# commaai/rednose

Measured on NVIDIA H100. Metric: fused EKF predict+update steps/s (batched, float64), higher is better.
Workload: dtype f64

## Files before the change

### rednose_b200/build.py

```python
import os
import shutil
import subprocess

PKG_DIR = os.path.dirname(os.path.abspath(__file__))
CSRC_DIR = os.path.join(PKG_DIR, "csrc")
INCLUDE_DIR = os.path.abspath(os.path.join(PKG_DIR, "..", "include"))
GENERATED_DIR = os.environ.get("REDNOSE_B200_GENERATED_DIR") or os.path.join(PKG_DIR, "generated")

NVCC_FLAGS = [
  "-gencode", "arch=compute_90a,code=sm_90a",
  "-O3", "-lineinfo", "-std=c++17", "--expt-relaxed-constexpr",
  "-Xcompiler", "-fPIC", "-shared",
]


def nvcc_path():
  p = shutil.which("nvcc") or "/usr/local/cuda/bin/nvcc"
  if not os.path.exists(p):
    raise RuntimeError("nvcc not found: rednose_b200 needs the CUDA toolkit to build filter libraries")
  return p


TUNE_ENV = ("REDNOSE_B200_GROUP", "REDNOSE_B200_WARPS", "REDNOSE_B200_TMA", "REDNOSE_B200_STAGES", "REDNOSE_B200_TMA_STORE", "REDNOSE_B200_SMALLSYM",
            "REDNOSE_B200_RTS_MMA", "REDNOSE_B200_MIN_WARPS", "REDNOSE_B200_PAIR", "REDNOSE_B200_PAIR_GROUP", "REDNOSE_B200_PAIR_MIN_WARPS",
            "REDNOSE_B200_RTS_MIN_CTAS", "REDNOSE_B200_CTA_MIN_BLOCKS", "REDNOSE_B200_PAIR_WAR_FIX", "REDNOSE_B200_PAIR_LATE_REFILL", "REDNOSE_B200_MAXRREG")


def _flags_match(folder, name):
  want = " ".join(f"{e}={os.environ[e]}" for e in TUNE_ENV if os.environ.get(e))
  try:
    with open(os.path.join(folder, f".{name}.env"), encoding="utf-8") as f:
      return f.read() == want
  except OSError:
    return want == ""


def _newer(target, sources):
  if not os.path.exists(target):
    return False
  t = os.path.getmtime(target)
  return all(os.path.getmtime(s) <= t for s in sources if os.path.exists(s))


def csrc_sources():
  return [os.path.join(CSRC_DIR, f) for f in sorted(os.listdir(CSRC_DIR)) if f != "runtime.cc"] + [os.path.join(INCLUDE_DIR, "rednose_b200.h")]


def compile_filter(folder, name, force=False, verbose=False):
  src = os.path.join(folder, f"{name}.cu")
  lib = os.path.join(folder, f"lib{name}.so")
  if not force and _newer(lib, [src] + csrc_sources()) and _flags_match(folder, name):
    return lib
  import fcntl
  with open(os.path.join(folder, f".{name}.lock"), "w") as lock:
    fcntl.flock(lock, fcntl.LOCK_EX)
    if not force and _newer(lib, [src] + csrc_sources()) and _flags_match(folder, name):
      return lib
    out = _compile_filter_locked(folder, name, src, lib, verbose)
    with open(os.path.join(folder, f".{name}.env"), "w", encoding="utf-8") as f:
      f.write(" ".join(f"{e}={os.environ[e]}" for e in TUNE_ENV if os.environ.get(e)))
    return out


def _compile_filter_locked(folder, name, src, lib, verbose):
  tune = [f"-D{k}={os.environ[e]}" for k, e in (("RNB_GROUP", "REDNOSE_B200_GROUP"), ("RNB_WARPS", "REDNOSE_B200_WARPS"), ("RNB_TMA", "REDNOSE_B200_TMA"), ("RNB_STAGES", "REDNOSE_B200_STAGES"), ("RNB_TMA_STORE", "REDNOSE_B200_TMA_STORE"), ("RNB_SMALLSYM", "REDNOSE_B200_SMALLSYM"), ("RNB_RTS_MMA", "REDNOSE_B200_RTS_MMA"), ("RNB_MIN_WARPS", "REDNOSE_B200_MIN_WARPS"), ("RNB_PAIR", "REDNOSE_B200_PAIR"), ("RNB_PAIR_GROUP", "REDNOSE_B200_PAIR_GROUP"), ("RNB_PAIR_MIN_WARPS", "REDNOSE_B200_PAIR_MIN_WARPS"), ("RNB_RTS_MIN_CTAS", "REDNOSE_B200_RTS_MIN_CTAS"), ("RNB_CTA_MIN_BLOCKS", "REDNOSE_B200_CTA_MIN_BLOCKS"), ("RNB_PAIR_WAR_FIX", "REDNOSE_B200_PAIR_WAR_FIX"), ("RNB_PAIR_LATE_REFILL", "REDNOSE_B200_PAIR_LATE_REFILL")) if os.environ.get(e)]
  if os.environ.get("REDNOSE_B200_MAXRREG"):
    tune += ["-maxrregcount", os.environ["REDNOSE_B200_MAXRREG"]]
  tmp = lib + f".tmp{os.getpid()}"
  cmd = [nvcc_path()] + NVCC_FLAGS + tune + ["-Xptxas", "-v", f"-I{CSRC_DIR}", f"-I{INCLUDE_DIR}", "-o", tmp, src]
  with open(os.path.join(folder, f".{name}.flags"), "w", encoding="utf-8") as f:
    f.write(" ".join(tune))
  res = subprocess.run(cmd, capture_output=True, text=True)
  with open(os.path.join(folder, f"{name}.ptxas.log"), "w", encoding="utf-8") as f:
    f.write(" ".join(cmd) + "\n" + res.stdout + res.stderr)
  if res.returncode != 0:
    raise RuntimeError(f"nvcc failed for {src}:\n{res.stderr[-4000:]}")
  os.replace(tmp, lib)
  if verbose:
    print(res.stderr)
  return lib


def compile_runtime(force=False):
  src = os.path.join(CSRC_DIR, "runtime.cc")
  lib = os.path.join(PKG_DIR, "librednose_b200.so")
  deps = [src, os.path.join(INCLUDE_DIR, "rednose_b200.h")]
  if not force and _newer(lib, deps):
    return lib
  import fcntl
  with open(os.path.join(PKG_DIR, ".runtime.lock"), "w") as lock:
    fcntl.flock(lock, fcntl.LOCK_EX)
    if not force and _newer(lib, deps):
      return lib
    cxx = shutil.which("g++") or "g++"
    tmp = lib + f".tmp{os.getpid()}"
    cmd = [cxx, "-O2", "-g", "-std=c++17", "-fPIC", "-shared", "-Wall", f"-I{INCLUDE_DIR}", "-o", tmp, src, "-ldl"]
    res = subprocess.run(cmd, capture_output=True, text=True)
    if res.returncode != 0:
      raise RuntimeError(f"g++ failed for {src}:\n{res.stderr[-4000:]}")
    os.replace(tmp, lib)
  return lib
```

### rednose_b200/codegen/symbolic.py

```python
from __future__ import annotations

import sympy as sp
from sympy.printing.c import C99CodePrinter


def normalise(expr):
  reps = {f: sp.Integer(int(f)) for f in expr.atoms(sp.Float) if abs(float(f)) <= 16.0 and float(f) == int(float(f))}
  return expr.xreplace(reps) if reps else expr


def _probe_value(e):
  from sympy.matrices.expressions.matexpr import MatrixElement
  reps = {}
  for a in e.atoms(MatrixElement) | e.atoms(sp.Symbol):
    if isinstance(a, sp.Symbol) and any(a in m.free_symbols for m in e.atoms(MatrixElement)):
      continue
    h = (hash(str(a)) % 9973) / 9973.0
    reps[a] = sp.Float(0.37 + 0.91 * h)
  try:
    v = complex(sp.N(e.xreplace(reps), 20))
  except (TypeError, ValueError):
    return None
  return abs(v)


def is_structural_zero(e, expand_limit=400):
  if e == 0 or e.is_zero:
    return True
  if e.is_number:
    return float(e) == 0.0
  v = _probe_value(e)
  if v is not None and v > 1e-9:
    return False
  if sp.count_ops(e) <= expand_limit:
    return sp.expand(e) == 0
  return False


class CudaPrinter(C99CodePrinter):

  def __init__(self, array_names: dict[str, str], scalar_names: dict[str, str]):
    super().__init__({'contract': False})
    self._arrays = array_names
    self._scalars = scalar_names

  def _print_MatrixElement(self, expr):
    parent = expr.parent
    cname = self._arrays.get(str(parent.name) if hasattr(parent, 'name') else str(parent))
    if cname is None:
      raise KeyError(f"matrix symbol {parent} is not an argument of this routine")
    idx = int(expr.i) * int(parent.shape[1]) + int(expr.j)
    return f"{cname}[{idx}]"

  def _print_Symbol(self, expr):
    return self._scalars.get(expr.name, expr.name)

  def _mul_chain(self, base: str, n: int) -> str:
    return "(" + "*".join([base] * n) + ")"

  def _print_Pow(self, expr):
    base, exp = expr.base, expr.exp
    if exp.is_number:
      e2 = sp.nsimplify(2 * exp) if not exp.is_Rational else 2 * exp
      if e2.is_Integer and abs(int(e2)) <= 16:
        twice = int(e2)
        b = self.parenthesize(base, 1000)
        n, half = divmod(abs(twice), 2)
        parts = []
        if n == 1:
          parts.append(b)
        elif n > 1:
          parts.append(self._mul_chain(b, n))
        if half:
          parts.append(f"sqrt({self._print(base)})")
        body = "*".join(parts) if parts else "1.0"
        if twice < 0:
          return f"(1.0/({body}))"
        return body if len(parts) == 1 else f"({body})"
    return f"pow({self._print(base)}, {self._print(exp)})"

  def _print_Integer(self, expr):
    return f"{int(expr)}.0"

  def _print_Rational(self, expr):
    return f"({int(expr.p)}.0/{int(expr.q)}.0)"


def cse_block(outputs: list[tuple[str, sp.Expr]], printer: CudaPrinter, tmp_prefix: str = "_c", indent: str = "    ") -> str:
  if not outputs:
    return ""
  exprs = [normalise(sp.sympify(e)) for _, e in outputs]
  repl, reduced = sp.cse(exprs, symbols=sp.numbered_symbols(tmp_prefix), optimizations='basic', order='none')
  lines = []
  for sym, e in repl:
    lines.append(f"{indent}const double {sym} = {printer.doprint(e)};")
  for (target, _), e in zip(outputs, reduced):
    lines.append(f"{indent}{target} = {printer.doprint(e)};")
  return "\n".join(lines) + "\n"


def sparse_pattern(mat: sp.Matrix):
  out = []
  for i in range(mat.shape[0]):
    for j in range(mat.shape[1]):
      e = normalise(mat[i, j])
      if not is_structural_zero(e):
        out.append((i, j, e))
  return out
```

### rednose_b200/csrc/ekf_warp2.cuh

```cuda
#pragma once
#include "ekf_warp.cuh"
#include "ekf_packed.cuh"
#include <cstdlib>

namespace rnb {

#ifndef RNB_PAIR
#define RNB_PAIR 1
#endif
#ifndef RNB_PAIR_GROUP
#define RNB_PAIR_GROUP 16
#endif
#ifndef RNB_PAIR_MIN_WARPS
#define RNB_PAIR_MIN_WARPS 8
#endif
#ifndef RNB_PAIR_FV_EARLY
#define RNB_PAIR_FV_EARLY 0
#endif
#ifndef RNB_PAIR_WAR_FIX
#define RNB_PAIR_WAR_FIX 1
#endif
#ifndef RNB_PAIR_LATE_REFILL
#define RNB_PAIR_LATE_REFILL 0
#endif
#ifndef RNB_PAIR_TMA_STAGE
#define RNB_PAIR_TMA_STAGE 1
#endif

template <bool PACKED>
constexpr int pair_stages() { return PACKED ? 2 : RNB_STAGES; }

template <class M, class K, int G, bool PACKED>
struct PairScratch {
  using L = RowLayout<M, K>;
  static constexpr int E = M::EDIM;
  static constexpr int NST = pair_stages<PACKED>();
  static constexpr int TS = PACKED ? packed_doubles(E) : E * E;
  alignas(128) double tile[NST * 2 * TS];
  alignas(8) uint64_t full[NST];
  alignas(16) double rows[G * L::STRIDE];
  static constexpr int EXS = ((E + 3) & ~3) + 2;
  static constexpr int HPS = 32;
  static constexpr int exrow(int sl) { return sl * EXS + 2 * (sl >> 3); }
  static constexpr int EXN = exrow(M::NFROWS > 0 ? M::NFROWS : 1) + 32;
  static constexpr int HPN = K::ZDIM * HPS;
  static constexpr int STG_X = 0;
  static constexpr int STG_Z = STG_X + even_up(G * M::DIM);
  static constexpr int STG_R = STG_Z + even_up(G * K::ZDIM);
  static constexpr int STG_DT = STG_R + even_up(G * K::ZDIM * K::ZDIM);
  static constexpr int STG_N = STG_DT + even_up(G);
  static constexpr int XN0 = ((EXN > HPN ? EXN : HPN) + 3) & ~1;
  static constexpr int XN1 = (STG_N + 1) / 2;
  static constexpr int XN = (((XN0 > XN1 ? XN0 : XN1) + 1) & ~1) | 2;
  alignas(16) double exhp[2 * XN];
  alignas(8) uint64_t stg;
};

template <class M, class K, bool PRED, bool UPD, int G, bool GATHER, bool PACKED>
__global__ void __launch_bounds__(32, RNB_PAIR_MIN_WARPS) ekf_step_pair(const StepArgs<M::NG> a) {
  constexpr int D = M::DIM, E = M::EDIM, Z = K::ZDIM;
  using L = RowLayout<M, K>;
  using SC = PairScratch<M, K, G, PACKED>;
  constexpr int RS = L::STRIDE, HPS = SC::HPS, XN = SC::XN;
  static_assert(E <= 32 && E % 2 == 0, "pair kernel: even EDIM <= 32");
  static_assert(G <= 32 && G % 2 == 0, "group size");
  extern __shared__ __align__(128) unsigned char smem_raw[];
  SC& s = *reinterpret_cast<SC*>(smem_raw);

  const int lane = threadIdx.x & 31;
  const long long b0 = (long long)blockIdx.x * G;
  if (b0 >= a.B) return;
  const int ng = (a.B - b0 < G) ? (int)(a.B - b0) : G;
  const int h = lane >> 4;
  const int hl_raw = lane & 15;
  const bool act = hl_raw < E / 2;
  const int hl = act ? hl_raw : E / 2 - 1;
  const int c0 = 2 * hl;
  double* myrow = s.rows + (lane < G ? lane : 0) * RS;
  const bool mine = lane < ng;
  long long myfid = b0 + (mine ? lane : 0);
  if constexpr (GATHER) { if (mine) myfid = (long long)a.idx[b0 + lane]; }
  auto fid_of = [&](int f) -> long long {
    if constexpr (GATHER) return __shfl_sync(0xffffffffu, myfid, f);
    else return b0 + f;
  };
  double* exh = s.exhp + h * XN;

  constexpr int NST = SC::NST;
  constexpr int TS = SC::TS;
  constexpr uint32_t TILE_BYTES = TS * sizeof(double);
  uint32_t it = 0;
  if (lane == 0) {
#pragma unroll
    for (int st = 0; st < NST; ++st) mbar_init(&s.full[st], 1);
    mbar_init(&s.stg, 1);
    asm volatile("fence.mbarrier_init.release.cluster;" ::: "memory");
    fence_async_smem();
  }
  __syncwarp();
  auto issue_pair = [&](int f, uint32_t slot, long long fidA, long long fidB) {
    const int np = (ng - f >= 2) ? 2 : 1;
    mbar_expect_tx(&s.full[slot], np * TILE_BYTES);
    double* dst = s.tile + slot * (2 * TS);
    if constexpr (GATHER) {
      tma_load_1d(dst, a.P + fidA * (long long)TS, TILE_BYTES, &s.full[slot]);
      if (np == 2) tma_load_1d(dst + TS, a.P + fidB * (long long)TS, TILE_BYTES, &s.full[slot]);
    } else {
      tma_load_1d(dst, a.P + fidA * (long long)TS, np * TILE_BYTES, &s.full[slot]);
    }
  };
  auto store_cols = [&](double* Pm, const double (&q0)[E], const double (&q1)[E]) {
#pragma unroll
    for (int i = 0; i < E; ++i) *reinterpret_cast<double2*>(Pm + i * E + c0) = make_double2(q0[i], q1[i]);
  };
  auto store_full = [&](double* Pm, const double (&q0)[E], const double (&q1)[E]) {
#pragma unroll
    for (int I = 0; I < E / 2; ++I) {
      if (I >= hl) {
        *reinterpret_cast<double2*>(Pm + 2 * I * E + c0) = make_double2(q0[2 * I], I == hl ? q0[2 * I + 1] : q1[2 * I]);
        *reinterpret_cast<double2*>(Pm + (2 * I + 1) * E + c0) = make_double2(q0[2 * I + 1], q1[2 * I + 1]);
      }
      if (I > hl) {
        *reinterpret_cast<double2*>(Pm + c0 * E + 2 * I) = make_double2(q0[2 * I], q0[2 * I + 1]);
        *reinterpret_cast<double2*>(Pm + (c0 + 1) * E + 2 * I) = make_double2(q1[2 * I], q1[2 * I + 1]);
      }
    }
  };

  double qd0 = 0.0, qd1 = 0.0;
  if (PRED && (a.flags & FLAG_Q_DIAG)) { qd0 = __ldg(a.Q + c0 * E + c0); qd1 = __ldg(a.Q + (c0 + 1) * E + c0 + 1); }

  const int n_obs = UPD ? a.n_obs : 1;
  for (int o = 0; o < n_obs; ++o) {
    const bool do_pred = PRED && o == 0;
    if (o > 0) {
      asm volatile("fence.proxy.async;" ::: "memory");
      __syncwarp();
    }
#pragma unroll
    for (int k = 0; k < NST; ++k) {
      const long long fa = fid_of(2 * k < ng ? 2 * k : 0), fb = fid_of(2 * k + 1 < ng ? 2 * k + 1 : 0);
      if (lane == 0 && 2 * k < ng) issue_pair(2 * k, (it + k) % NST, fa, fb);
    }

    double dt_lane = a.dt;
    bool staged = false;
    if constexpr (RNB_PAIR_TMA_STAGE && !GATHER) {
      const bool ok = o == 0 && ng == G && (!UPD || a.n_obs == 1) &&
          !((reinterpret_cast<uintptr_t>(a.x) | reinterpret_cast<uintptr_t>(a.z) | reinterpret_cast<uintptr_t>(a.R) |
             reinterpret_cast<uintptr_t>(a.dt_arr)) & 15u);
      if (ok) {
        staged = true;
        const bool shared_R = UPD && (a.flags & FLAG_SHARED_R);
        const bool want_dt = do_pred && a.dt_arr;
        double* stg = s.exhp;
        if (lane == 0) {
          uint32_t bytes = G * D * 8;
          if (UPD) bytes += G * Z * 8 + (shared_R ? 0 : G * Z * Z * 8);
          if (want_dt) bytes += G * 8;
          mbar_expect_tx(&s.stg, bytes);
          tma_load_1d(stg + SC::STG_X, a.x + b0 * D, G * D * 8, &s.stg);
          if (UPD) {
            tma_load_1d(stg + SC::STG_Z, a.z + b0 * Z, G * Z * 8, &s.stg);
            if (!shared_R) tma_load_1d(stg + SC::STG_R, a.R + b0 * (Z * Z), G * Z * Z * 8, &s.stg);
          }
          if (want_dt) tma_load_1d(stg + SC::STG_DT, a.dt_arr + b0, G * 8, &s.stg);
        }
        mbar_wait(&s.stg, 0);
        if (mine) {
#pragma unroll
          for (int i = 0; i < D; ++i) myrow[L::OFF_X + i] = stg[SC::STG_X + lane * D + i];
          if constexpr (UPD) {
#pragma unroll
            for (int i = 0; i < Z; ++i) myrow[L::OFF_Y + i] = stg[SC::STG_Z + lane * Z + i];
#pragma unroll
            for (int i = 0; i < Z * Z; ++i) myrow[L::OFF_R + i] = shared_R ? __ldg(a.R + i) : stg[SC::STG_R + lane * (Z * Z) + i];
          }
          if (want_dt) dt_lane = stg[SC::STG_DT + lane];
        }
      }
    }
    if (!staged) {
      StageRegs<D, G> rx;
      StageRegs<Z, G> rz;
      StageRegs<Z * Z, G> rR;
      const bool shared_R = UPD && (a.flags & FLAG_SHARED_R);
      const bool bulk_obs = UPD && a.n_obs == 1;
      if (o == 0) {
        if (GATHER) gather_load<D, G>(a.x, rx, ng, lane, myfid);
        else stage_load<D, G>(a.x + b0 * D, rx, ng, lane);
      }
      if constexpr (UPD) {
        if (bulk_obs) {
          stage_load<Z, G>(a.z + b0 * Z, rz, ng, lane);
          if (!shared_R) stage_load<Z * Z, G>(a.R + b0 * (Z * Z), rR, ng, lane);
        }
      }
      if (do_pred && mine && a.dt_arr) dt_lane = a.dt_arr[b0 + lane];
      if (o == 0) stage_store<D, RS, G>(rx, s.rows, L::OFF_X, ng, lane);
      if constexpr (UPD) {
        if (bulk_obs) {
          stage_store<Z, RS, G>(rz, s.rows, L::OFF_Y, ng, lane);
          if (!shared_R) stage_store<Z * Z, RS, G>(rR, s.rows, L::OFF_R, ng, lane);
        } else if (mine) {
          const long long bo = (b0 + lane) * a.n_obs + o;
#pragma unroll
          for (int i = 0; i < Z; ++i) myrow[L::OFF_Y + i] = a.z[bo * Z + i];
          if (!shared_R) {
#pragma unroll
            for (int i = 0; i < Z * Z; ++i) myrow[L::OFF_R + i] = a.R[bo * (Z * Z) + i];
          }
        }
        if (shared_R && mine) {
#pragma unroll
          for (int i = 0; i < Z * Z; ++i) myrow[L::OFF_R + i] = __ldg(a.R + i);
        }
      }
    }
    __syncwarp();

    if (mine) {
      double xp[L::Dp];
      vec_load(myrow + L::OFF_X, xp);
      if (do_pred) {
        double fv[L::NFp];
        double xn[L::Dp];
        M::predict_leaf(xp, dt_lane, a.gv, xn, fv);
        if constexpr (L::NFp > M::NF) fv[L::NFp - 1] = 0.0;
        if constexpr (L::Dp > D) xn[L::Dp - 1] = 0.0;
        vec_store(myrow + L::OFF_FV, fv);
        myrow[L::OFF_DT] = dt_lane;
        vec_store(myrow + L::OFF_X, xn);
        if ((a.flags & FLAG_NORM_AFTER_PREDICT) && a.n_quat > 0) lane_normalize(myrow + L::OFF_X, a);
        vec_load(myrow + L::OFF_X, xp);
      }
      if constexpr (UPD) {
        const double* ea = a.ea ? a.ea + ((b0 + lane) * a.n_obs + o) * a.ea_dim : nullptr;
        double hx[Z];
        double hv[L::NHp];
        K::obs_leaf(xp, ea, a.gv, hx, hv);
        if constexpr (L::NHp > K::NH) hv[L::NHp - 1] = 0.0;
        vec_store(myrow + L::OFF_HV, hv);
#pragma unroll
        for (int i = 0; i < Z; ++i) myrow[L::OFF_Y + i] -= hx[i];
      }
    }
    __syncwarp();
    if (do_pred && a.hx_pred) {
      if (GATHER) scatter_out<D, RS>(a.hx_pred, s.rows, L::OFF_X, ng, lane, myfid);
      else stage_out<D, RS>(a.hx_pred + b0 * D, s.rows, L::OFF_X, ng, lane);
    }
    if constexpr (UPD) {
      if (a.n_obs == 1) {
        stage_out<Z, RS>(a.z + b0 * Z, s.rows, L::OFF_Y, ng, lane);
      } else if (mine) {
        const long long bo = (b0 + lane) * a.n_obs + o;
#pragma unroll
        for (int i = 0; i < Z; ++i) a.z[bo * Z + i] = myrow[L::OFF_Y + i];
      }
    }

#pragma unroll 1
    for (int f = 0; f < ng; f += 2) {
      const bool valid = f + h < ng;
      const int fi = valid ? f + h : f;
      const bool wr = valid && act;
      const long long b = fid_of(fi);
      double* row = s.rows + fi * RS;
      const uint32_t slot = it % NST;
      const double* tile = s.tile + slot * (2 * TS) + (valid ? h : 0) * TS;
      double p0[E], p1[E];
      double fv[L::NFp];
      if (RNB_PAIR_FV_EARLY && do_pred) vec_load(row + L::OFF_FV, fv);

      mbar_wait(&s.full[slot], (it / NST) & 1u);
#pragma unroll
      for (int I = 0; I < E / 2; ++I) {
        const int mx = I > hl ? I : hl, mn = I > hl ? hl : I;
        const double* pb = tile + (PACKED ? packed_block(mx, mn) : 2 * mx * E + 2 * mn);
        const double2 u = *reinterpret_cast<const double2*>(pb);
        const double2 v = *reinterpret_cast<const double2*>(pb + (PACKED ? 2 : E));
        p0[2 * I] = u.x;
        p1[2 * I] = I > hl ? u.y : v.x;
        p0[2 * I + 1] = I >= hl ? v.x : u.y;
        p1[2 * I + 1] = v.y;
      }
      const int fn = f + 2 * NST;
      const long long fa = fid_of(fn < ng ? fn : 0), fb = fid_of(fn + 1 < ng ? fn + 1 : 0);
      constexpr bool LATE = RNB_PAIR_LATE_REFILL && (M::NFROWS > 0);
      if (!(LATE && do_pred)) {
        if constexpr (RNB_PAIR_WAR_FIX & 1) fence_async_smem();
        if constexpr (RNB_PAIR_WAR_FIX & 2) {
          const double landed = p0[E - 1] + p1[E - 1];
          asm volatile("" ::"d"(landed));
        }
        __syncwarp();
        if (lane == 0 && fn < ng) issue_pair(fn, slot, fa, fb);
      }
      ++it;

      if (do_pred) {
        if (!RNB_PAIR_FV_EARLY) vec_load(row + L::OFF_FV, fv);
        const double dt = row[L::OFF_DT];
        if constexpr (M::NFROWS > 0) {
          {
            double m0[E], m1[E];
#pragma unroll
            for (int i = 0; i < E; ++i) { m0[i] = p0[i]; m1[i] = p1[i]; }
            M::F_apply(fv, m0);
            M::F_apply(fv, m1);
            if (act) {
              int sl = 0;
#pragma unroll
              for (int r = 0; r < E; ++r) {
                if ((M::FROW_MASK >> r) & 1u) {
                  *reinterpret_cast<double2*>(exh + SC::exrow(sl) + c0) = make_double2(m0[r], m1[r]);
                  ++sl;
                }
              }
            }
          }
          if constexpr (LATE) fence_async_smem();
          __syncwarp();
          if constexpr (LATE) { if (lane == 0 && fn < ng) issue_pair(fn, slot, fa, fb); }
          if ((M::FROW_MASK >> c0) & 1u) {
            const double* xr = exh + SC::exrow(__popc(M::FROW_MASK & ((1u << c0) - 1u)));
#pragma unroll
            for (int i = 0; i < E; ++i) p0[i] = xr[i];
          }
          if ((M::FROW_MASK >> (c0 + 1)) & 1u) {
            const double* xr = exh + SC::exrow(__popc(M::FROW_MASK & ((2u << c0) - 1u)));
#pragma unroll
            for (int i = 0; i < E; ++i) p1[i] = xr[i];
          }
          M::F_apply(fv, p0);
          M::F_apply(fv, p1);
          __syncwarp();
        } else {
          M::F_apply(fv, p0);
          M::F_apply(fv, p1);
        }
        if (a.flags & FLAG_Q_DIAG) {
          const double dq0 = dt * qd0, dq1 = dt * qd1;
#pragma unroll
          for (int i = 0; i < E; i += 2) {
            asm("{\n .reg .pred q;\n setp.eq.s32 q, %2, %3;\n @q add.f64 %0, %0, %1;\n}" : "+d"(p0[i]) : "d"(dq0), "r"(c0), "r"(i));
            asm("{\n .reg .pred q;\n setp.eq.s32 q, %2, %3;\n @q add.f64 %0, %0, %1;\n}" : "+d"(p1[i + 1]) : "d"(dq1), "r"(c0), "r"(i));
          }
        } else {
          const double* Qg = a.Q + c0;
#pragma unroll
          for (int i = 0; i < E; ++i) {
            p0[i] = fma(dt, __ldg(Qg + i * E), p0[i]);
            p1[i] = fma(dt, __ldg(Qg + i * E + 1), p1[i]);
          }
        }
        if (a.hP_pred && wr) store_cols(a.hP_pred + b * (long long)(E * E), p0, p1);
      }

      if constexpr (UPD) {
        double hp0[Z], hp1[Z];
        double S[Z][Z];
        {
          double hv[L::NHp];
          vec_load(row + L::OFF_HV, hv);
          K::Herr_apply(hv, p0, hp0);
          K::Herr_apply(hv, p1, hp1);
#pragma unroll
          for (int c = 0; c < Z; ++c) {
            if (hl_raw < HPS / 2)
              *reinterpret_cast<double2*>(exh + c * HPS + 2 * hl_raw) = act ? make_double2(hp0[c], hp1[c]) : make_double2(0.0, 0.0);
          }
          __syncwarp();
#pragma unroll
          for (int i = 0; i < Z; ++i)
#pragma unroll
            for (int j = 0; j < Z; ++j) S[i][j] = 0.0;
          K::S_accum(hv, [&](int c, int k) { return exh[c * HPS + k]; }, S);
        }
        double y[L::Zp], R[L::ZZp];
        vec_load(row + L::OFF_Y, y);
        vec_load(row + L::OFF_R, R);

        SolverZ<Z> ldl;
        if constexpr (K::MAHA) {
          double Sg[Z][Z];
#pragma unroll
          for (int i = 0; i < Z; ++i)
#pragma unroll
            for (int j = 0; j < Z; ++j) Sg[i][j] = S[i][j] + R[i * Z + j];
          ldl.factor(Sg);
          double u[Z];
#pragma unroll
          for (int i = 0; i < Z; ++i) u[i] = y[i];
          ldl.solve(u);
          double d = 0.0;
#pragma unroll
          for (int i = 0; i < Z; ++i) d += y[i] * u[i];
          const double infl = (d > K::MAHA_THRESH) ? 1.0e16 : 1.0;
#pragma unroll
          for (int i = 0; i < Z * Z; ++i) R[i] *= infl;
        }
#pragma unroll
        for (int i = 0; i < Z; ++i)
#pragma unroll
          for (int j = 0; j < Z; ++j) S[i][j] += R[i * Z + j];
        ldl.factor(S);

        ldl.solve(hp0);
        ldl.solve(hp1);
        double dx0 = 0.0, dx1 = 0.0;
#pragma unroll
        for (int c = 0; c < Z; ++c) { dx0 = fma(hp0[c], y[c], dx0); dx1 = fma(hp1[c], y[c], dx1); }
        if (wr) *reinterpret_cast<double2*>(row + L::OFF_FV + c0) = make_double2(dx0, dx1);

#pragma unroll
        for (int i = 0; i < E; i += 2) {
          double a0 = p0[i], a1 = p0[i + 1], b0v = p1[i], b1v = p1[i + 1];
#pragma unroll
          for (int c = 0; c < Z; ++c) {
            const double2 h2 = *reinterpret_cast<const double2*>(exh + c * HPS + i);
            a0 = fma(-h2.x, hp0[c], a0);
            a1 = fma(-h2.y, hp0[c], a1);
            b0v = fma(-h2.x, hp1[c], b0v);
            b1v = fma(-h2.y, hp1[c], b1v);
          }
          p0[i] = a0; p0[i + 1] = a1; p1[i] = b0v; p1[i + 1] = b1v;
        }
        __syncwarp();
        if (a.hP_filt && wr && o == n_obs - 1) store_full(a.hP_filt + b * (long long)(E * E), p0, p1);
      }

      if (wr) {
        if constexpr (PACKED) {
          double* Pg = a.P + b * (long long)TS;
#pragma unroll
          for (int I = 0; I < E / 2; ++I) {
            if (I >= hl) {
              double* q = Pg + packed_block(I, hl);
              *reinterpret_cast<double2*>(q) = make_double2(p0[2 * I], I == hl ? p0[2 * I + 1] : p1[2 * I]);
              *reinterpret_cast<double2*>(q + 2) = make_double2(p0[2 * I + 1], p1[2 * I + 1]);
            }
          }
        } else {
          store_full(a.P + b * (long long)(E * E), p0, p1);
        }
      }
    }
    __syncwarp();

    if constexpr (UPD) {
      if (mine) {
        double xp[L::Dp], dx[L::Ep], xn[L::Dp];
        vec_load(myrow + L::OFF_X, xp);
        vec_load(myrow + L::OFF_FV, dx);
        M::err_fun(xp, dx, a.gv, xn);
        if constexpr (L::Dp > D) xn[L::Dp - 1] = 0.0;
        vec_store(myrow + L::OFF_X, xn);
        if ((a.flags & FLAG_NORM_AFTER_UPDATE) && a.n_quat > 0) lane_normalize(myrow + L::OFF_X, a);
      }
      __syncwarp();
    }
    if (o == n_obs - 1) {
      if (GATHER) scatter_out<D, RS>(a.x, s.rows, L::OFF_X, ng, lane, myfid);
      else stage_out<D, RS>(a.x + b0 * D, s.rows, L::OFF_X, ng, lane);
      if (UPD && a.hx_filt) {
        if (GATHER) scatter_out<D, RS>(a.hx_filt, s.rows, L::OFF_X, ng, lane, myfid);
        else stage_out<D, RS>(a.hx_filt + b0 * D, s.rows, L::OFF_X, ng, lane);
      }
    }
    __syncwarp();
  }
}

template <class M, class K, int G, bool PACKED>
constexpr size_t pair_smem_bytes() { return sizeof(PairScratch<M, K, G, PACKED>); }

template <class M>
constexpr bool use_pair() { return RNB_PAIR && RNB_TMA && M::EDIM % 2 == 0 && M::EDIM <= 32; }

inline bool pair_enabled() {
  const char* e = getenv("REDNOSE_B200_WARP_KERNEL");
  return !(e && e[0] == 's');
}

}
```

Baseline: 568.4 million.

## Issue staging TMA before tile prefetch, fuse sincos, simplify tile indexing, add profiling

The bulk TMA loads for x, z, R and dt are now issued before the per-pair covariance tile prefetches, so the staging transfer starts earlier and overlaps with them. The code generator now emits sincos() for arguments that need both sin and cos, replacing two separate transcendental calls. The per-iteration block-offset computation in the tile unpack loop is simplified using precomputed per-lane bases. An optional clock64 phase profiler is also added behind a compile flag that is off by default.

New measurement: 582.1 million, median of 6. 1.02x the previous value.

```diff
diff --git a/rednose_b200/build.py b/rednose_b200/build.py
--- a/rednose_b200/build.py
+++ b/rednose_b200/build.py
@@ -23,7 +23,8 @@
 
 TUNE_ENV = ("REDNOSE_B200_GROUP", "REDNOSE_B200_WARPS", "REDNOSE_B200_TMA", "REDNOSE_B200_STAGES", "REDNOSE_B200_TMA_STORE", "REDNOSE_B200_SMALLSYM",
             "REDNOSE_B200_RTS_MMA", "REDNOSE_B200_MIN_WARPS", "REDNOSE_B200_PAIR", "REDNOSE_B200_PAIR_GROUP", "REDNOSE_B200_PAIR_MIN_WARPS",
-            "REDNOSE_B200_RTS_MIN_CTAS", "REDNOSE_B200_CTA_MIN_BLOCKS", "REDNOSE_B200_PAIR_WAR_FIX", "REDNOSE_B200_PAIR_LATE_REFILL", "REDNOSE_B200_MAXRREG")
+            "REDNOSE_B200_RTS_MIN_CTAS", "REDNOSE_B200_CTA_MIN_BLOCKS", "REDNOSE_B200_PAIR_WAR_FIX", "REDNOSE_B200_PAIR_LATE_REFILL", "REDNOSE_B200_MAXRREG",
+            "REDNOSE_B200_PAIR_PROFILE")
 
 
 def _flags_match(folder, name):
@@ -63,7 +64,7 @@
 
 
 def _compile_filter_locked(folder, name, src, lib, verbose):
-  tune = [f"-D{k}={os.environ[e]}" for k, e in (("RNB_GROUP", "REDNOSE_B200_GROUP"), ("RNB_WARPS", "REDNOSE_B200_WARPS"), ("RNB_TMA", "REDNOSE_B200_TMA"), ("RNB_STAGES", "REDNOSE_B200_STAGES"), ("RNB_TMA_STORE", "REDNOSE_B200_TMA_STORE"), ("RNB_SMALLSYM", "REDNOSE_B200_SMALLSYM"), ("RNB_RTS_MMA", "REDNOSE_B200_RTS_MMA"), ("RNB_MIN_WARPS", "REDNOSE_B200_MIN_WARPS"), ("RNB_PAIR", "REDNOSE_B200_PAIR"), ("RNB_PAIR_GROUP", "REDNOSE_B200_PAIR_GROUP"), ("RNB_PAIR_MIN_WARPS", "REDNOSE_B200_PAIR_MIN_WARPS"), ("RNB_RTS_MIN_CTAS", "REDNOSE_B200_RTS_MIN_CTAS"), ("RNB_CTA_MIN_BLOCKS", "REDNOSE_B200_CTA_MIN_BLOCKS"), ("RNB_PAIR_WAR_FIX", "REDNOSE_B200_PAIR_WAR_FIX"), ("RNB_PAIR_LATE_REFILL", "REDNOSE_B200_PAIR_LATE_REFILL")) if os.environ.get(e)]
+  tune = [f"-D{k}={os.environ[e]}" for k, e in (("RNB_GROUP", "REDNOSE_B200_GROUP"), ("RNB_WARPS", "REDNOSE_B200_WARPS"), ("RNB_TMA", "REDNOSE_B200_TMA"), ("RNB_STAGES", "REDNOSE_B200_STAGES"), ("RNB_TMA_STORE", "REDNOSE_B200_TMA_STORE"), ("RNB_SMALLSYM", "REDNOSE_B200_SMALLSYM"), ("RNB_RTS_MMA", "REDNOSE_B200_RTS_MMA"), ("RNB_MIN_WARPS", "REDNOSE_B200_MIN_WARPS"), ("RNB_PAIR", "REDNOSE_B200_PAIR"), ("RNB_PAIR_GROUP", "REDNOSE_B200_PAIR_GROUP"), ("RNB_PAIR_MIN_WARPS", "REDNOSE_B200_PAIR_MIN_WARPS"), ("RNB_RTS_MIN_CTAS", "REDNOSE_B200_RTS_MIN_CTAS"), ("RNB_CTA_MIN_BLOCKS", "REDNOSE_B200_CTA_MIN_BLOCKS"), ("RNB_PAIR_WAR_FIX", "REDNOSE_B200_PAIR_WAR_FIX"), ("RNB_PAIR_LATE_REFILL", "REDNOSE_B200_PAIR_LATE_REFILL"), ("RNB_PAIR_PROFILE", "REDNOSE_B200_PAIR_PROFILE")) if os.environ.get(e)]
   if os.environ.get("REDNOSE_B200_MAXRREG"):
     tune += ["-maxrregcount", os.environ["REDNOSE_B200_MAXRREG"]]
   tmp = lib + f".tmp{os.getpid()}"
diff --git a/rednose_b200/codegen/symbolic.py b/rednose_b200/codegen/symbolic.py
--- a/rednose_b200/codegen/symbolic.py
+++ b/rednose_b200/codegen/symbolic.py
@@ -86,15 +86,44 @@
     return f"({int(expr.p)}.0/{int(expr.q)}.0)"
 
 
+def _sincos_pairs(repl, reduced, tmp_prefix):
+  exprs = [e for _, e in repl] + list(reduced)
+  atoms = set().union(*(e.atoms(sp.sin, sp.cos) for e in exprs)) if exprs else set()
+  args = sorted({f.args[0] for f in atoms if isinstance(f, sp.sin)} & {f.args[0] for f in atoms if isinstance(f, sp.cos)},
+                key=sp.default_sort_key)
+  own = {e: sym for sym, e in repl if isinstance(e, (sp.sin, sp.cos)) and e.args[0] in args}
+  fresh = sp.numbered_symbols(tmp_prefix + "s")
+  pairs = {a: (own.get(sp.sin(a)) or next(fresh), own.get(sp.cos(a)) or next(fresh)) for a in args}
+  subs = {}
+  for a, (s, c) in pairs.items():
+    subs[sp.sin(a)], subs[sp.cos(a)] = s, c
+  return pairs, subs, set(own.values())
+
+
 def cse_block(outputs: list[tuple[str, sp.Expr]], printer: CudaPrinter, tmp_prefix: str = "_c", indent: str = "    ") -> str:
   if not outputs:
     return ""
   exprs = [normalise(sp.sympify(e)) for _, e in outputs]
   repl, reduced = sp.cse(exprs, symbols=sp.numbered_symbols(tmp_prefix), optimizations='basic', order='none')
+  pairs, subs, dropped = _sincos_pairs(repl, reduced, tmp_prefix)
+  pending = dict(pairs)
   lines = []
+
+  def emit_sincos(syms):
+    for a, (s, c) in list(pending.items()):
+      if s in syms or c in syms:
+        lines.append(f"{indent}double {s}, {c};")
+        lines.append(f"{indent}sincos({printer.doprint(a)}, &{s}, &{c});")
+        del pending[a]
+
   for sym, e in repl:
-    lines.append(f"{indent}const double {sym} = {printer.doprint(e)};")
+    e = e.xreplace(subs)
+    emit_sincos(e.free_symbols | {sym})
+    if sym not in dropped:
+      lines.append(f"{indent}const double {sym} = {printer.doprint(e)};")
   for (target, _), e in zip(outputs, reduced):
+    e = e.xreplace(subs)
+    emit_sincos(e.free_symbols)
     lines.append(f"{indent}{target} = {printer.doprint(e)};")
   return "\n".join(lines) + "\n"
 
diff --git a/rednose_b200/csrc/ekf_warp2.cuh b/rednose_b200/csrc/ekf_warp2.cuh
--- a/rednose_b200/csrc/ekf_warp2.cuh
+++ b/rednose_b200/csrc/ekf_warp2.cuh
@@ -25,6 +25,17 @@
 #endif
 #ifndef RNB_PAIR_TMA_STAGE
 #define RNB_PAIR_TMA_STAGE 1
+#endif
+#ifndef RNB_PAIR_PROFILE
+#define RNB_PAIR_PROFILE 0
+#endif
+
+#if RNB_PAIR_PROFILE
+enum : int { PROF_STAGE, PROF_A, PROF_WAIT, PROF_PAIR, PROF_C, PROF_OUT, PROF_GROUPS, PROF_N };
+__device__ unsigned long long rnb_pair_prof[PROF_N];
+#define RNB_PROF_MARK(ph) do { const long long t_ = clock64(); prof_[ph] += (unsigned)(t_ - tprev_); tprev_ = t_; } while (0)
+#else
+#define RNB_PROF_MARK(ph) do {} while (0)
 #endif
 
 template <bool PACKED>
@@ -70,12 +81,18 @@
   const int lane = threadIdx.x & 31;
   const long long b0 = (long long)blockIdx.x * G;
   if (b0 >= a.B) return;
+#if RNB_PAIR_PROFILE
+  unsigned prof_[PROF_N] = {};
+  long long tprev_ = clock64();
+#endif
   const int ng = (a.B - b0 < G) ? (int)(a.B - b0) : G;
   const int h = lane >> 4;
   const int hl_raw = lane & 15;
   const bool act = hl_raw < E / 2;
   const int hl = act ? hl_raw : E / 2 - 1;
   const int c0 = 2 * hl;
+  const int blk_below = PACKED ? packed_block(0, hl) : c0;
+  const int blk_above = PACKED ? packed_block(hl, 0) : c0 * E;
   double* myrow = s.rows + (lane < G ? lane : 0) * RS;
   const bool mine = lane < ng;
   long long myfid = b0 + (mine ? lane : 0);
@@ -137,35 +154,35 @@
       asm volatile("fence.proxy.async;" ::: "memory");
       __syncwarp();
     }
+    double dt_lane = a.dt;
+    bool staged = false;
+    const bool shared_R = UPD && (a.flags & FLAG_SHARED_R);
+    const bool want_dt = do_pred && a.dt_arr;
+    double* stg = s.exhp;
+    if constexpr (RNB_PAIR_TMA_STAGE && !GATHER) {
+      staged = o == 0 && ng == G && (!UPD || a.n_obs == 1) &&
+          !((reinterpret_cast<uintptr_t>(a.x) | reinterpret_cast<uintptr_t>(a.z) | reinterpret_cast<uintptr_t>(a.R) |
+             reinterpret_cast<uintptr_t>(a.dt_arr)) & 15u);
+      if (staged && lane == 0) {
+        uint32_t bytes = G * D * 8;
+        if (UPD) bytes += G * Z * 8 + (shared_R ? 0 : G * Z * Z * 8);
+        if (want_dt) bytes += G * 8;
+        mbar_expect_tx(&s.stg, bytes);
+        tma_load_1d(stg + SC::STG_X, a.x + b0 * D, G * D * 8, &s.stg);
+        if (UPD) {
+          tma_load_1d(stg + SC::STG_Z, a.z + b0 * Z, G * Z * 8, &s.stg);
+          if (!shared_R) tma_load_1d(stg + SC::STG_R, a.R + b0 * (Z * Z), G * Z * Z * 8, &s.stg);
+        }
+        if (want_dt) tma_load_1d(stg + SC::STG_DT, a.dt_arr + b0, G * 8, &s.stg);
+      }
+    }
 #pragma unroll
     for (int k = 0; k < NST; ++k) {
       const long long fa = fid_of(2 * k < ng ? 2 * k : 0), fb = fid_of(2 * k + 1 < ng ? 2 * k + 1 : 0);
       if (lane == 0 && 2 * k < ng) issue_pair(2 * k, (it + k) % NST, fa, fb);
     }
-
-    double dt_lane = a.dt;
-    bool staged = false;
     if constexpr (RNB_PAIR_TMA_STAGE && !GATHER) {
-      const bool ok = o == 0 && ng == G && (!UPD || a.n_obs == 1) &&
-          !((reinterpret_cast<uintptr_t>(a.x) | reinterpret_cast<uintptr_t>(a.z) | reinterpret_cast<uintptr_t>(a.R) |
-             reinterpret_cast<uintptr_t>(a.dt_arr)) & 15u);
-      if (ok) {
-        staged = true;
-        const bool shared_R = UPD && (a.flags & FLAG_SHARED_R);
-        const bool want_dt = do_pred && a.dt_arr;
-        double* stg = s.exhp;
-        if (lane == 0) {
-          uint32_t bytes = G * D * 8;
-          if (UPD) bytes += G * Z * 8 + (shared_R ? 0 : G * Z * Z * 8);
-          if (want_dt) bytes += G * 8;
-          mbar_expect_tx(&s.stg, bytes);
-          tma_load_1d(stg + SC::STG_X, a.x + b0 * D, G * D * 8, &s.stg);
-          if (UPD) {
-            tma_load_1d(stg + SC::STG_Z, a.z + b0 * Z, G * Z * 8, &s.stg);
-            if (!shared_R) tma_load_1d(stg + SC::STG_R, a.R + b0 * (Z * Z), G * Z * Z * 8, &s.stg);
-          }
-          if (want_dt) tma_load_1d(stg + SC::STG_DT, a.dt_arr + b0, G * 8, &s.stg);
-        }
+      if (staged) {
         mbar_wait(&s.stg, 0);
         if (mine) {
 #pragma unroll
@@ -184,7 +201,6 @@
       StageRegs<D, G> rx;
       StageRegs<Z, G> rz;
       StageRegs<Z * Z, G> rR;
-      const bool shared_R = UPD && (a.flags & FLAG_SHARED_R);
       const bool bulk_obs = UPD && a.n_obs == 1;
       if (o == 0) {
         if (GATHER) gather_load<D, G>(a.x, rx, ng, lane, myfid);
@@ -218,6 +234,7 @@
       }
     }
     __syncwarp();
+    RNB_PROF_MARK(PROF_STAGE);
 
     if (mine) {
       double xp[L::Dp];
@@ -259,6 +276,7 @@
         for (int i = 0; i < Z; ++i) a.z[bo * Z + i] = myrow[L::OFF_Y + i];
       }
     }
+    RNB_PROF_MARK(PROF_A);
 
 #pragma unroll 1
     for (int f = 0; f < ng; f += 2) {
@@ -273,11 +291,13 @@
       double fv[L::NFp];
       if (RNB_PAIR_FV_EARLY && do_pred) vec_load(row + L::OFF_FV, fv);
 
+      RNB_PROF_MARK(PROF_PAIR);
       mbar_wait(&s.full[slot], (it / NST) & 1u);
+      RNB_PROF_MARK(PROF_WAIT);
 #pragma unroll
       for (int I = 0; I < E / 2; ++I) {
-        const int mx = I > hl ? I : hl, mn = I > hl ? hl : I;
-        const double* pb = tile + (PACKED ? packed_block(mx, mn) : 2 * mx * E + 2 * mn);
+        const double* pb = tile + (I > hl ? blk_below + (PACKED ? packed_block(I, 0) : 2 * I * E)
+                                          : blk_above + (PACKED ? packed_block(0, I) : 2 * I));
         const double2 u = *reinterpret_cast<const double2*>(pb);
         const double2 v = *reinterpret_cast<const double2*>(pb + (PACKED ? 2 : E));
         p0[2 * I] = u.x;
@@ -448,6 +468,7 @@
       }
     }
     __syncwarp();
+    RNB_PROF_MARK(PROF_PAIR);
 
     if constexpr (UPD) {
       if (mine) {
@@ -461,6 +482,7 @@
       }
       __syncwarp();
     }
+    RNB_PROF_MARK(PROF_C);
     if (o == n_obs - 1) {
       if (GATHER) scatter_out<D, RS>(a.x, s.rows, L::OFF_X, ng, lane, myfid);
       else stage_out<D, RS>(a.x + b0 * D, s.rows, L::OFF_X, ng, lane);
@@ -470,8 +492,28 @@
       }
     }
     __syncwarp();
+    RNB_PROF_MARK(PROF_OUT);
   }
+#if RNB_PAIR_PROFILE
+  if (lane == 0) {
+    prof_[PROF_GROUPS] = 1;
+#pragma unroll
+    for (int i = 0; i < PROF_N; ++i) atomicAdd(&rnb_pair_prof[i], (unsigned long long)prof_[i]);
+  }
+#endif
 }
+
+#if RNB_PAIR_PROFILE
+extern "C" int rnb_pair_profile_read(unsigned long long* out, int reset) {
+  cudaError_t e = cudaDeviceSynchronize();
+  if (e == cudaSuccess) e = cudaMemcpyFromSymbol(out, rnb_pair_prof, sizeof(unsigned long long) * PROF_N);
+  if (e == cudaSuccess && reset) {
+    const unsigned long long zero[PROF_N] = {};
+    e = cudaMemcpyToSymbol(rnb_pair_prof, zero, sizeof(zero));
+  }
+  return (int)e;
+}
+#endif
 
 template <class M, class K, int G, bool PACKED>
 constexpr size_t pair_smem_bytes() { return sizeof(PairScratch<M, K, G, PACKED>); }
```
